# gplepage/lsqfit

Hardware: AMD Instinct MI355X
Metric: fp64 LM steps/sec at (N_data,N_param)=(65536,4096); chi2 match vs GSL (higher is better)
Workload: dtype f64

## Files before the change

lsqfit_amd/csrc/chol.hip:

```cpp
#include <cstdlib>

#include "common.h"

namespace lsqamd {

constexpr int NB = CHOL_NB;
constexpr int PLD = NB + 2;
constexpr int SB = 32;

typedef double v4d __attribute__((ext_vector_type(4)));
typedef double v2d __attribute__((ext_vector_type(2)));

size_t potrf_work_bytes(int64_t n) {
  const int64_t nblk = (n + NB - 1) / NB;
  return (size_t)nblk * NB * NB * sizeof(double);
}

__device__ __forceinline__ double readlane_d(double v, int lane) {
  union { double d; int i[2]; } u;
  u.d = v;
  u.i[0] = __builtin_amdgcn_readlane(u.i[0], lane);
  u.i[1] = __builtin_amdgcn_readlane(u.i[1], lane);
  return u.d;
}


constexpr int WLD = SB + 2;

__device__ __forceinline__ double rsqrt_refined(double d) {
  double y = __builtin_amdgcn_rsq(d);
  const double h = -0.5 * d;
  double e = __builtin_fma(h * y, y, 0.5);
  y = __builtin_fma(y, e, y);
  e = __builtin_fma(h * y, y, 0.5);
  return __builtin_fma(y, e, y);
}

__device__ __noinline__ void chol32_wave(double *s, int j0, double *dinv, double *wbuf,
                                         int32_t *info, int k0, int lane) {
  const int c = lane & 31;
  const bool isW = lane >= SB;
  double col[SB];
#pragma unroll
  for (int i = 0; i < SB; ++i) col[i] = s[(j0 + i) * PLD + j0 + c];
#pragma unroll
  for (int i = 0; i < SB; ++i) col[i] = isW ? ((i == c) ? 1.0 : 0.0) : col[i];
  int first_bad = -1;
  double d = readlane_d(col[0], 0);
  bool ok = (d > 0.0) && (d < 1.0e300);
  first_bad = ok ? first_bad : 0;
  double y = rsqrt_refined(ok ? d : 1.0);
  double ykeep = 0.0;
#pragma unroll
  for (int j = 0; j < SB; ++j) {
    double u = col[j] * y;
    u = (!isW && c < j) ? 0.0 : u;
    col[j] = u;
    ykeep = (c == j) ? y : ykeep;
    double ynext = 0.0;
    if (j + 1 < SB) {
      const double dn = readlane_d(col[j + 1] - u * u, j + 1);
      ok = (dn > 0.0) && (dn < 1.0e300);
      first_bad = (!ok && first_bad < 0) ? j + 1 : first_bad;
      ynext = rsqrt_refined(ok ? dn : 1.0);
    }
#pragma unroll
    for (int i0 = j + 1; i0 < SB; i0 += 8) {
      double ub[8];
// ... 200 lines not shown
    }
  }
  STAMP(17);
  {
    const int c2 = (tid & 63) * 2, rg = tid >> 6;
    for (int it = 0; it < 32; ++it) {
      const int r = it * 4 + rg;
      if (r >= nb) continue;
      v2d v = *reinterpret_cast<const v2d *>(s + r * PLD + c2);
      v.x = (c2 >= r && c2 < nb) ? v.x : 0.0;
      v.y = (c2 + 1 >= r && c2 + 1 < nb) ? v.y : 0.0;
      *reinterpret_cast<v2d *>(uinv + r * NB + c2) = v;
    }
  }
  STAMP(18);
}

static PerDeviceOnce g_potf2_attr;
long long *g_potf2_dbg = nullptr;
static constexpr size_t POTF2_LDS = (size_t)(NB * PLD + NB + SB * WLD) * sizeof(double);

static hipError_t launch_potf2(hipStream_t st, double *A, int64_t lda, int nb, double *uinv,
                               int32_t *info, int32_t k0, int32_t batch = 1, int64_t strideA = 0,
                               int64_t strideW = 0, const int32_t *active = nullptr) {
  {
    const hipError_t ea = g_potf2_attr.run([] {
      hipError_t e = hipFuncSetAttribute(reinterpret_cast<const void *>(potf2_inv_kernel<true>),
                                         hipFuncAttributeMaxDynamicSharedMemorySize, (int)POTF2_LDS);
      if (e != hipSuccess) return e;
      return hipFuncSetAttribute(reinterpret_cast<const void *>(potf2_inv_kernel<false>),
                                 hipFuncAttributeMaxDynamicSharedMemorySize, (int)POTF2_LDS);
    });
    if (ea != hipSuccess) return ea;
  }
  static const bool use_mfma = [] {
    const char *e = getenv("LSQAMD_POTF2");
    return !(e && e[0] == 'l');
  }();
  if (use_mfma) {
    return launch_potf2_mfma(st, A, lda, nb, uinv, info, k0, batch, strideA, strideW, active);
  }
  const bool vec = !(lda & 1) && !(reinterpret_cast<uintptr_t>(A) & 15) && !(strideA & 1);
  if (vec)
    hipLaunchKernelGGL(potf2_inv_kernel<true>, dim3((unsigned)batch), dim3(256), POTF2_LDS, st, A, lda, nb,
                       uinv, info, k0, g_potf2_dbg, strideA, strideW, active);
  else
    hipLaunchKernelGGL(potf2_inv_kernel<false>, dim3((unsigned)batch), dim3(256), POTF2_LDS, st, A, lda, nb,
                       uinv, info, k0, g_potf2_dbg, strideA, strideW, active);
  return hipGetLastError();
}

hipError_t potrf_upper_batched(hipStream_t st, double *A, int64_t n, int64_t lda, int64_t n_cols,
                               double *work, int32_t *dev_info, int32_t batch, int64_t strideA,
                               int64_t strideW, const int32_t *active, bool info_zeroed) {
  hipError_t e = info_zeroed ? hipSuccess : hipMemsetAsync(dev_info, 0, sizeof(int32_t) * (size_t)batch, st);
  if (e != hipSuccess) return e;
  static const int64_t fuse_min_tiles = [] { const char *v = getenv("LSQAMD_FUSE_MIN_TILES"); return v ? atoll(v) : (int64_t)10; }();
  const bool can_fuse = batch == 1 && !active && fuse_min_tiles >= 0 && trail_potf2_available() && (n % NB) == 0 &&
                        (n_cols % NB) == 0 &&
                        !(lda & 1) && !(reinterpret_cast<uintptr_t>(A) & 15);
  bool diag_done = false;
  for (int64_t k0 = 0; k0 < n; k0 += NB) {
    const int nb = (int)((n - k0) < NB ? (n - k0) : NB);
    double *uinv = work + (k0 / NB) * NB * NB;
    if (!diag_done) {
      e = launch_potf2(st, A + k0 * lda + k0, lda, nb, uinv, dev_info, (int32_t)k0, batch, strideA, strideW,
                       active);
      if (e != hipSuccess) return e;
    }
    diag_done = false;
    const int64_t rest = n_cols - (k0 + nb);
    if (rest <= 0) continue;
    GemmTN p;
    p.X = uinv; p.ldx = NB; p.sx = strideW;
    p.Y = A + k0 * lda + k0 + nb; p.ldy = lda; p.sy = strideA;
    p.C = A + k0 * lda + k0 + nb; p.ldc = lda; p.sc = strideA;
    p.M = nb; p.N = rest; p.K = nb;
    p.x_upper_tri = 1;
    p.batch = batch; p.batch_active = active;
    e = launch_gemm_tn(st, p);
    if (e != hipSuccess) return e;
    const int64_t mrest = n - (k0 + nb);
    if (mrest <= 0) continue;
    const int64_t tiles = (mrest / NB) * (mrest / NB + 1) / 2;
    if (can_fuse && tiles >= fuse_min_tiles) {
      e = launch_trail_potf2(st, p.C, A + (k0 + nb) * lda + (k0 + nb), lda, mrest, rest, NB,
                             work + ((k0 + nb) / NB) * NB * NB, dev_info, (int32_t)(k0 + nb));
      if (e != hipSuccess) return e;
      diag_done = true;
      continue;
    }
    GemmTN t;
    t.X = p.C; t.ldx = lda; t.sx = strideA;
    t.Y = p.C; t.ldy = lda; t.sy = strideA;
    t.C = A + (k0 + nb) * lda + (k0 + nb); t.ldc = lda; t.sc = strideA;
    t.M = mrest; t.N = rest; t.K = nb;
    t.alpha = -1.0; t.beta = 1.0;
    t.upper_only = 1;
    t.batch = batch; t.batch_active = active;
    e = launch_gemm_tn(st, t);
    if (e != hipSuccess) return e;
  }
  return hipSuccess;
}

hipError_t potrf_upper(hipStream_t st, double *A, int64_t n, int64_t lda, int64_t n_cols,
                       double *work, int32_t *dev_info, bool info_zeroed) {
  return potrf_upper_batched(st, A, n, lda, n_cols, work, dev_info, 1, 0, 0, nullptr, info_zeroed);
}

constexpr int BS_ROWS = 16;

__device__ __forceinline__ double wave_sum(double v) {
#pragma unroll
  for (int o = 32; o > 0; o >>= 1) v += __shfl_down(v, o, 64);
  return v;
}

__global__ __launch_bounds__(256) void backsolve_step_kernel(const double *A, int64_t lda, int64_t k0,
                                                             int nb, const double *uinv, double *y,
                                                             double *v, int64_t strideA, int64_t strideW,
                                                             int64_t strideY, const int32_t *active) {
  if (active && !active[blockIdx.y]) return;
  A += (int64_t)blockIdx.y * strideA;
  uinv += (int64_t)blockIdx.y * strideW;
  y += (int64_t)blockIdx.y * strideY;
  v += (int64_t)blockIdx.y * strideY;
  __shared__ double vk[NB];
  __shared__ double yk[NB];
  const int tid = threadIdx.x, lane = tid & 63, wave = tid >> 6;
  if (tid < NB) yk[tid] = tid < nb ? y[k0 + tid] : 0.0;
  double a0[32], a1[32];
#pragma unroll
  for (int i = 0; i < 32; ++i) {
    const int r = wave * 32 + i;
    const bool ok = r < nb;
    a0[i] = (ok && lane < nb) ? uinv[r * NB + lane] : 0.0;
    a1[i] = (ok && lane + 64 < nb) ? uinv[r * NB + lane + 64] : 0.0;
  }
  __syncthreads();
  const double y0 = yk[lane], y1 = yk[lane + 64];
#pragma unroll
  for (int i = 0; i < 32; ++i) {
    const double acc = wave_sum(a0[i] * y0 + a1[i] * y1);
    if (lane == 0) vk[wave * 32 + i] = acc;
  }
  __syncthreads();
  if (blockIdx.x == 0) {
    if (tid < nb) v[k0 + tid] = vk[tid];
    return;
  }
  const int64_t r0 = (int64_t)(blockIdx.x - 1) * BS_ROWS + wave * (BS_ROWS / 4);
  double u0[BS_ROWS / 4], u1[BS_ROWS / 4];
#pragma unroll
  for (int i = 0; i < BS_ROWS / 4; ++i) {
    const int64_t r = r0 + i;
    const bool ok = r < k0;
    const double *row = A + (ok ? r : 0) * lda + k0;
    u0[i] = (ok && lane < nb) ? row[lane] : 0.0;
    u1[i] = (ok && lane + 64 < nb) ? row[lane + 64] : 0.0;
  }
// ... 396 lines not shown
```

lsqfit_amd/csrc/common.h:

```cpp
#pragma once
#include <hip/hip_runtime.h>
#include <stddef.h>
#include <stdint.h>

#include <atomic>
#include <cstdio>
#include <exception>
#include <mutex>
#include <new>

#include "../../include/lsqfit_amd.h"

namespace lsqamd {

struct lsqamd_abi_no_handle { const char *err; };

template <class H> int abi_exception(H *h) noexcept {
  int code = LSQAMD_EINTERNAL;
  char buf[320];
  std::snprintf(buf, sizeof buf, "internal error: unknown C++ exception caught at the C ABI");
  try {
    throw;
  } catch (const std::bad_alloc &) {
    code = LSQAMD_ENOMEM;
// ... 69 lines not shown
  }
};

struct GemmTN {
  const double *X = nullptr, *Y = nullptr;
  double *C = nullptr;
  int64_t M = 0, N = 0, K = 0;
  int64_t ldx = 0, ldy = 0, ldc = 0;
  double alpha = 1.0, beta = 0.0;
  int32_t batch = 1;
  int64_t sx = 0, sy = 0, sc = 0;
  int32_t upper_only = 0;
  int32_t x_upper_tri = 0;
  int32_t xy_lower_tri = 0;
  int32_t splits = 1;
  int64_t split_stride = 0;
  const int32_t *work_map = nullptr;
  int32_t n_work = 0;
  int32_t force_generic = 0;
  const int32_t *batch_active = nullptr;
  int32_t tri_halves = 0;
  double *colsum_out = nullptr;
  int64_t colsum_ld = 0, colsum_rcol = 0;
  int32_t *done_ctr = nullptr;
};
bool gemm_tn_fuses_colsum(const GemmTN &g);
bool gemm_tn_wants_tri_halves(const GemmTN &g);
hipError_t launch_gemm_tn(hipStream_t st, const GemmTN &g);
struct WhitenSynth {
  int32_t model = 0;
  const double *Wt = nullptr;
  const double *x = nullptr;
  const double *p = nullptr;
  double *J = nullptr;
  int64_t ld = 0, B = 0, K = 0;
  int32_t nb = 0;
  double *colsum_out = nullptr;
  const int32_t *trig_far = nullptr;
};
bool whiten_synth_eligible(int32_t model, int64_t B, int64_t P);
hipError_t launch_whiten_synth(hipStream_t st, const WhitenSynth &a);
int64_t syrk_work_count(int64_t P, int32_t splits);
void syrk_work_fill(int64_t P, int32_t splits, int32_t *out);
int64_t syrk_work_fill_rows(int64_t P, int32_t splits, int row0, int row1, int32_t *out);
void syrk_work_fill_grouped(int64_t P, int32_t splits, int G, const int32_t *rows, int32_t *out, int32_t *count);
hipError_t launch_wait_counter(hipStream_t st, const int32_t *ctr, int32_t expect, int32_t *timed_out);

constexpr int CHOL_NB = 128;
size_t potrf_work_bytes(int64_t n);
hipError_t potrf_upper(hipStream_t st, double *A, int64_t n, int64_t lda, int64_t n_cols,
                       double *work, int32_t *dev_info, bool info_zeroed = false);
bool trail_potf2_available();
hipError_t launch_trail_potf2(hipStream_t st, const double *P, double *C, int64_t lda, int64_t mrest,
                              int64_t rest, int nb_next, double *uinv_next, int32_t *info, int32_t k0_next);
hipError_t launch_potf2_mfma(hipStream_t st, double *A, int64_t lda, int nb, double *uinv, int32_t *info,
                             int32_t k0, int32_t batch, int64_t strideA, int64_t strideW,
                             const int32_t *active);

hipError_t potrf_upper_batched(hipStream_t st, double *A, int64_t n, int64_t lda, int64_t n_cols,
                               double *work, int32_t *dev_info, int32_t batch, int64_t strideA,
                               int64_t strideW, const int32_t *active, bool info_zeroed = false);
hipError_t backsolve_upper_batched(hipStream_t st, const double *A, int64_t n, int64_t lda,
                                   const double *work, double *y_inout, int32_t batch, int64_t strideA,
                                   int64_t strideW, int64_t strideY, const int32_t *active,
                                   void *scratch = nullptr, int32_t *info_dev = nullptr, bool scratch_zeroed = false);
hipError_t trtri_upper_to_lower_T_batched(hipStream_t st, const double *A, int64_t n, int64_t lda,
                                          const double *work, double *Wl, int64_t ldw, int32_t batch,
                                          int64_t strideA, int64_t strideW, int64_t strideWl);
size_t backsolve_scratch_bytes(int64_t n);
hipError_t backsolve_upper(hipStream_t st, const double *A, int64_t n, int64_t lda,
                           const double *work, double *y_inout, void *scratch = nullptr, int32_t *info_dev = nullptr,
                           bool scratch_zeroed = false);
hipError_t trtri_upper_to_lower_T(hipStream_t st, const double *A, int64_t n, int64_t lda,
                                  const double *work, double *Wl, int64_t ldw);
hipError_t logdiag_sum(hipStream_t st, const double *A, int64_t n, int64_t lda, double *dev_out);
extern long long *g_potf2_dbg;

struct TapeProgram {
  int64_t row0 = 0, n_rows = 0;
  int32_t tape_off = 0, n_tape = 0;
  const void *jit = nullptr;
};
struct ModelArgs {
  int32_t model = 0;
  int64_t n_data = 0, n_param = 0;
  int32_t n_x = 0;
  const double *x = nullptr;
  const double *ymean = nullptr;
  const double *wdiag = nullptr;
  const uint8_t *in_block = nullptr;
  const double *p = nullptr;
  const int32_t *tape = nullptr;
  int32_t n_tape = 0;
  const double *consts = nullptr;
  int32_t n_batch = 1;
  int64_t p_stride = 0, out_stride = 0;
  int64_t ymean_stride = 0;
  int64_t wdiag_stride = 0;
  const int32_t *batch_active = nullptr;
  const int32_t *trig_far = nullptr;
  const int32_t *tape_poff = nullptr;
  double *tape_part = nullptr;
  double *tape_jt = nullptr;
  int64_t tape_ldn = 0, tape_wgs = 0;
  int32_t tape_slots = 0;
  const int32_t *tape_seg = nullptr;
  int32_t tape_n_seg = 0, tape_seg_depth = 0, tape_seg_slots = 0, tape_slot_cap = 0, tape_single = 0;
  const void *jit = nullptr;
  const TapeProgram *progs = nullptr;
  int32_t n_prog = 0;
};
int tape_slots_of_op(int op);
hipError_t launch_trig_range(hipStream_t st, const double *q, int64_t n, double xmax, int32_t *flag);
hipError_t launch_residual_ex(hipStream_t st, const ModelArgs &m, double *r_w, double *r_raw);
// ... 125 lines not shown
```

lsqfit_amd/csrc/gemm_tn_f64.hip:

```cpp
#include <cstdlib>

#include "common.h"
#include <type_traits>
#include <vector>
#include "devmath.h"

namespace lsqamd {

#ifdef LSQAMD_SYRK_STAMPS
__device__ unsigned long long *g_syrk_stamps = nullptr;
#endif

typedef double v4d __attribute__((ext_vector_type(4)));
typedef double v2d __attribute__((ext_vector_type(2)));

constexpr int BM = 128, BN = 128, BK = 16;
constexpr int LDT = BM + 16;
constexpr int STAGE = 2 * BK * LDT;
constexpr size_t GEMM_LDS_BYTES = 2 * STAGE * sizeof(double);

struct GemmDev {
  const double *X, *Y;
  double *C;
  int64_t M, N, K, ldx, ldy, ldc;
// ... 574 lines not shown
      for (int j = 0; j < 2; ++j) bb[j] = Ys[kr * LDS_S + wn * 32 + j * 16 + fr];
#pragma unroll
      for (int i = 0; i < 2; ++i)
#pragma unroll
        for (int j = 0; j < 2; ++j)
          acc[i][j] = __builtin_amdgcn_mfma_f64_16x16x4f64(a[i], bb[j], acc[i][j], 0, 0, 0);
    }
    if (more) sstore(cur ^ 1, k0 + BK);
    __syncthreads();
    cur ^= 1;
  }
  const double alpha = g.alpha;
  const double beta = g.splits > 1 ? 0.0 : g.beta;
  double cv[2][2][4];
  if (beta != 0.0) {
#pragma unroll
    for (int i = 0; i < 2; ++i)
#pragma unroll
      for (int j = 0; j < 2; ++j)
#pragma unroll
        for (int r = 0; r < 4; ++r) {
          const int64_t col = n0 + wn * 32 + j * 16 + fr;
          const int64_t row = m0 + wm * 32 + i * 16 + fq + 4 * r;
          const bool ok = col < g.N && row < g.M;
          cv[i][j][r] = C[(ok ? row : 0) * g.ldc + (ok ? col : 0)];
        }
  }
#pragma unroll
  for (int i = 0; i < 2; ++i)
#pragma unroll
    for (int j = 0; j < 2; ++j) {
      const int64_t col = n0 + wn * 32 + j * 16 + fr;
      if (col >= g.N) continue;
#pragma unroll
      for (int r = 0; r < 4; ++r) {
        const int64_t row = m0 + wm * 32 + i * 16 + fq + 4 * r;
        if (row >= g.M) continue;
        double v = alpha * acc[i][j][r];
        if (beta != 0.0) v += beta * cv[i][j][r];
        C[row * g.ldc + col] = v;
      }
    }
}

constexpr int PN = 64;
constexpr int LDS_PX = BM + 16;
constexpr int LDS_PY = PN + 16;
constexpr int STAGE_P = BK * (LDS_PX + LDS_PY);
constexpr size_t GEMM_LDS_BYTES_P = 2 * STAGE_P * sizeof(double);

constexpr int OS_LDX = 136, OS_PN = 16;
constexpr size_t GEMM_LDS_BYTES_OS = (size_t)(128 * OS_LDX + 128 * OS_PN) * sizeof(double);

__global__ __launch_bounds__(256) void gemm_tn_f64_panel_oneshot_kernel(GemmDev g) {
  extern __shared__ __attribute__((aligned(16))) double smem[];
  typedef __attribute__((address_space(3))) void lds_void;
  typedef const __attribute__((address_space(1))) void glb_void;
  const int tid = threadIdx.x, lane = tid & 63, wave = tid >> 6;
  const int64_t b = blockIdx.z;
  if (g.batch_active && !g.batch_active[b]) return;
  const double *X = g.X + b * g.sx;
  const int64_t n0 = (int64_t)blockIdx.x * OS_PN;
  double *Yg = g.C + b * g.sc + n0;
  double *Xs = smem, *Ys = smem + 128 * OS_LDX;
#pragma unroll 8
  for (int i = 0; i < 32; ++i) {
    const int k = wave * 32 + i;
    __builtin_amdgcn_global_load_lds((glb_void *)(X + (int64_t)k * g.ldx + 2 * lane), (lds_void *)(Xs + k * OS_LDX), 16, 0, 0);
  }
#pragma unroll
  for (int i = 0; i < 4; ++i) {
    const int k8 = (wave * 4 + i) * 8;
    __builtin_amdgcn_global_load_lds((glb_void *)(Yg + (int64_t)(k8 + (lane >> 3)) * g.ldc + 2 * (lane & 7)),
                                     (lds_void *)(Ys + k8 * OS_PN), 16, 0, 0);
  }
  __syncthreads();
  const int col = lane & 15, q = lane >> 4;
  const int i0 = wave, i1 = 7 - wave;
  v4d acc0 = {0.0, 0.0, 0.0, 0.0}, acc1 = {0.0, 0.0, 0.0, 0.0};
  const int n0c = 4 * (i0 + 1), n1c = 4 * (i1 + 1);
#pragma unroll 4
  for (int kc = 0; kc < n1c; ++kc) {
    const double bb = Ys[(4 * kc + q) * OS_PN + col];
    const double a1 = Xs[(4 * kc + q) * OS_LDX + 16 * i1 + col];
    acc1 = __builtin_amdgcn_mfma_f64_16x16x4f64(a1, bb, acc1, 0, 0, 0);
    if (kc < n0c) {
      const double a0 = Xs[(4 * kc + q) * OS_LDX + 16 * i0 + col];
      acc0 = __builtin_amdgcn_mfma_f64_16x16x4f64(a0, bb, acc0, 0, 0, 0);
    }
  }
#pragma unroll
  for (int r = 0; r < 4; ++r) {
    Yg[(int64_t)(16 * i0 + 4 * r + q) * g.ldc + col] = acc0[r];
    Yg[(int64_t)(16 * i1 + 4 * r + q) * g.ldc + col] = acc1[r];
  }
}

template <bool VEC, int PNW>
__global__ __launch_bounds__(256, 2) void gemm_tn_f64_panel_kernel(GemmDev g) {
  constexpr int WN = PNW >= 32 ? 2 : 1, WM = 4 / WN;
  constexpr int RW = BM / WM, NI = RW / 16;
  constexpr int CW = PNW / WN, NJ = CW / 16;
  constexpr int YT = PNW / 2, YROWS = 256 / YT;
  constexpr int YP = (BK + YROWS - 1) / YROWS;
  constexpr int LDY = PNW + 16;
  extern __shared__ __attribute__((aligned(16))) double smem[];
  const int tid = threadIdx.x;
  const int lane = tid & 63, wave = tid >> 6;
  const int wm = WN == 2 ? wave >> 1 : wave, wn = WN == 2 ? wave & 1 : 0;
  const int64_t m0 = 0, n0 = (int64_t)blockIdx.x * PNW;
  const int64_t b = blockIdx.z;
  if (g.batch_active && !g.batch_active[b]) return;
  const double *X = g.X + b * g.sx;
  const double *Y = g.Y + b * g.sy;
  double *C = g.C + b * g.sc;
  int64_t kb = 0, ke = g.K;
  if (g.x_upper_tri && ke > BM) ke = BM;
  v4d acc[NI][NJ];
#pragma unroll
  for (int i = 0; i < NI; ++i)
#pragma unroll
    for (int j = 0; j < NJ; ++j) acc[i][j] = (v4d){0.0, 0.0, 0.0, 0.0};
  const int xc2 = (tid & 63) * 2, xrg = tid >> 6;
  const int yc2 = (tid % YT) * 2, yrg = tid / YT;
  const int64_t xc = m0 + xc2, yc = n0 + yc2;
  const bool x0ok = xc < g.M, x1ok = xc + 1 < g.M;
  const bool y0ok = yc < g.N, y1ok = yc + 1 < g.N;
  const int64_t xi0 = VEC ? (xc < g.ldx - 2 ? xc : g.ldx - 2) : (xc < g.M ? xc : g.M - 1);
  const int64_t xi1 = xc + 1 < g.M ? xc + 1 : g.M - 1;
  const int64_t yi0 = VEC ? (yc < g.ldy - 2 ? yc : g.ldy - 2) : (yc < g.N ? yc : g.N - 1);
  const int64_t yi1 = yc + 1 < g.N ? yc + 1 : g.N - 1;
  v2d xr[4], yr[YP];
  auto gload = [&](int64_t k0) {
#pragma unroll
    for (int i = 0; i < 4; ++i) {
      int64_t row = k0 + xrg + 4 * i;
      row = row < ke ? row : ke - 1;
      xr[i] = load2<VEC>(X + row * g.ldx, xi0, xi1);
    }
#pragma unroll
    for (int i = 0; i < YP; ++i) {
      int64_t row = k0 + yrg + YROWS * i;
      row = row < ke ? row : ke - 1;
      yr[i] = load2<VEC>(Y + row * g.ldy, yi0, yi1);
    }
  };
  auto sstore = [&](int buf, int64_t k0) {
    double *Xs = smem + buf * STAGE_P;
// ... 622 lines not shown
```

lsqfit_amd/csrc/potf2_mfma.hip:

```cpp
#include <cstdlib>

#include "common.h"

#ifndef LSQAMD_LEAF_FMA_LAYOUT
#define LSQAMD_LEAF_FMA_LAYOUT 1
#endif

namespace lsqamd {

constexpr int NB = CHOL_NB;
typedef double v4d __attribute__((ext_vector_type(4)));

__device__ __forceinline__ double readlane_d(double v, int lane) {
  union { double d; int i[2]; } u;
  u.d = v;
  u.i[0] = __builtin_amdgcn_readlane(u.i[0], lane);
  u.i[1] = __builtin_amdgcn_readlane(u.i[1], lane);
  return u.d;
}

__device__ __forceinline__ double rsqrt_refined(double d) {
  double y = __builtin_amdgcn_rsq(d);
  const double h = -0.5 * d;
  double e = __builtin_fma(h * y, y, 0.5);
// ... 756 lines not shown
  }
}

template <int U>
__device__ __forceinline__ void tile_wave4(double *A, int64_t lda, int nb, double *uinv, Leaf4Shared &sh, int lane) {
  TileRegs4 T;
  load_tiles4<U>(T, A, lda, nb, lane);
  zero_upper_inv<U>(uinv, lane);
  Slab4Loop<0, U>::run(T, sh, A, lda, nb, uinv, lane);
}

__device__ __forceinline__ void potf2v4_run(double *A, int64_t lda, int nb, double *uinv, int32_t *info, int32_t k0,
                                            Leaf4Shared &sh, int tid) {
  const int lane = tid & 63;
  const int wave = __builtin_amdgcn_readfirstlane(tid >> 6);
  if (tid < 8) {
    sh.flagD[tid] = 0;
    sh.flagW[tid] = 0;
    sh.cnt[tid] = 0;
  }
  __syncthreads();
  if (wave == 0) pivot_wave4<true>(sh, A, lda, uinv, info, k0, nb, lane);
  else if (wave == 1) tile_wave4<0>(A, lda, nb, uinv, sh, lane);
  else if (wave == 2) tile_wave4<1>(A, lda, nb, uinv, sh, lane);
  else tile_wave4<2>(A, lda, nb, uinv, sh, lane);
}

__global__ __launch_bounds__(256) void potf2_v4_kernel(double *A, int64_t lda, int nb, double *uinv, int32_t *info,
                                                       int32_t k0, int64_t strideA, int64_t strideW,
                                                       const int32_t *active, long long *dbg) {
  __shared__ Leaf4Shared sh;
  if (active && !active[blockIdx.x]) return;
  A += (int64_t)blockIdx.x * strideA;
  uinv += (int64_t)blockIdx.x * strideW;
  info += blockIdx.x;
#ifdef LSQAMD_POTF2_TIMING
  if (threadIdx.x == 0) sh.stamps[60] = (long long)__builtin_readcyclecounter();
#endif
  potf2v4_run(A, lda, nb, uinv, info, k0, sh, threadIdx.x);
#ifdef LSQAMD_POTF2_TIMING
  __syncthreads();
  if (threadIdx.x == 0) sh.stamps[63] = (long long)__builtin_readcyclecounter();
  __syncthreads();
  if (dbg && threadIdx.x < 64) dbg[threadIdx.x] = sh.stamps[threadIdx.x];
#endif
}

struct TrailArgs {
  const double *P;
  double *C;
  int64_t lda;
  int32_t tiles_m, tiles_n;
  int32_t halves;
};

constexpr int TBK = 16, TLD = 128 + 16, TSTAGE = 2 * TBK * TLD;
constexpr size_t TRAIL_LDS_BYTES = 2 * TSTAGE * sizeof(double);

template <int NJ>
__device__ __forceinline__ void trail_tile(const TrailArgs &t, int tm, int tn, int half, double *smem, int tid) {
  const int lane = tid & 63, wave = tid >> 6;
  const int wm = wave >> 1, wn = wave & 1;
  const int64_t m0 = (int64_t)tm * 128, n0 = (int64_t)tn * 128;
  const int cw = (NJ == 4 ? 0 : 64 * half) + wn * 16 * NJ;
  v4d acc[4][NJ];
#pragma unroll
  for (int i = 0; i < 4; ++i)
#pragma unroll
    for (int j = 0; j < NJ; ++j) acc[i][j] = (v4d){0.0, 0.0, 0.0, 0.0};
  typedef __attribute__((address_space(3))) void lds_void;
  typedef const __attribute__((address_space(1))) void glb_void;
  const double *xp = t.P + (int64_t)wave * t.lda + m0 + 2 * lane;
  const double *yp = t.P + (int64_t)wave * t.lda + n0 + 2 * lane;
  const int64_t step4 = 4 * t.lda;
  auto stage = [&](int buf) {
    double *Xs = smem + buf * TSTAGE + wave * TLD;
    double *Ys = Xs + TBK * TLD;
#pragma unroll
    for (int i = 0; i < 4; ++i) {
      __builtin_amdgcn_global_load_lds((glb_void *)(xp + i * step4), (lds_void *)(Xs + 4 * i * TLD), 16, 0, 0);
      __builtin_amdgcn_global_load_lds((glb_void *)(yp + i * step4), (lds_void *)(Ys + 4 * i * TLD), 16, 0, 0);
    }
    xp += 4 * step4;
    yp += 4 * step4;
  };
  const int fr = lane & 15, fq = lane >> 4;
  stage(0);
  __syncthreads();
  int cur = 0;
  for (int k0 = 0; k0 < 128; k0 += TBK) {
    if (k0 + TBK < 128) stage(cur ^ 1);
    const double *Xs = smem + cur * TSTAGE;
    const double *Ys = Xs + TBK * TLD;
#pragma unroll
    for (int kk = 0; kk < TBK / 4; ++kk) {
      const int kr = kk * 4 + fq;
      double a[4], bb[NJ];
#pragma unroll
      for (int i = 0; i < 4; ++i) a[i] = Xs[kr * TLD + wm * 64 + i * 16 + fr];
#pragma unroll
      for (int j = 0; j < NJ; ++j) bb[j] = Ys[kr * TLD + cw + j * 16 + fr];
#pragma unroll
      for (int i = 0; i < 4; ++i)
#pragma unroll
        for (int j = 0; j < NJ; ++j) acc[i][j] = mfma4(a[i], bb[j], acc[i][j]);
    }
    __syncthreads();
    cur ^= 1;
  }
#pragma unroll
  for (int i = 0; i < 4; ++i) {
    double cv[NJ][4];
#pragma unroll
    for (int j = 0; j < NJ; ++j)
#pragma unroll
      for (int r = 0; r < 4; ++r)
        cv[j][r] = t.C[(m0 + wm * 64 + i * 16 + fq + 4 * r) * t.lda + n0 + cw + j * 16 + fr];
#pragma unroll
    for (int j = 0; j < NJ; ++j)
#pragma unroll
      for (int r = 0; r < 4; ++r)
        t.C[(m0 + wm * 64 + i * 16 + fq + 4 * r) * t.lda + n0 + cw + j * 16 + fr] = cv[j][r] - acc[i][j][r];
  }
}

constexpr int DLD4 = 128 + 8;
constexpr int DIAG4_HELP_OFF = 128 * DLD4;
constexpr size_t DIAG4_LDS_BYTES = (size_t)(128 * DLD4 + 9 * 4 * 64) * sizeof(double);
constexpr int v4_help_skip(int U) { return U == 1 ? 4 : (U == 2 ? 5 : 0); }

template <int U>
__device__ __forceinline__ void diag_update_from_panel4(TileRegs4 &T, const double *Ps, int lane) {
  const int col = lane & 15, q = lane >> 4;
#pragma unroll 4
  for (int kc = 0; kc < 32; ++kc) {
    const double *row = Ps + (4 * kc + q) * DLD4 + col;
    double a[8];
#pragma unroll
    for (int ti = 0; ti < 8; ++ti) a[ti] = -row[16 * ti];
#pragma unroll
    for (int c = 0; c < 3; ++c) {
      if (v4_has(U, c)) {
        const int tj = v4_col(U, c);
        const double b = row[16 * tj];
#pragma unroll
        for (int ti = 0; ti < 8; ++ti) {
          if (ti < tj && !(c == 2 && ti < v4_help_skip(U))) T.X[c][ti] = mfma4(a[ti], b, T.X[c][ti]);
          if (ti == tj) T.DA[c] = mfma4(a[ti], b, T.DA[c]);
        }
      }
    }
  }
}

__device__ __forceinline__ void diag_update_help4(double *Ps, int lane) {
  const int col = lane & 15, q = lane >> 4;
  const v4d zero = {0.0, 0.0, 0.0, 0.0};
  v4d h[9];
#pragma unroll
  for (int i = 0; i < 9; ++i) h[i] = zero;
#pragma unroll 4
  for (int kc = 0; kc < 32; ++kc) {
    const double *row = Ps + (4 * kc + q) * DLD4 + col;
    double a[5];
#pragma unroll
    for (int ti = 0; ti < 5; ++ti) a[ti] = -row[16 * ti];
    const double b6 = row[16 * 6], b5 = row[16 * 5];
#pragma unroll
    for (int ti = 0; ti < 4; ++ti) h[ti] = mfma4(a[ti], b6, h[ti]);
#pragma unroll
    for (int ti = 0; ti < 5; ++ti) h[4 + ti] = mfma4(a[ti], b5, h[4 + ti]);
  }
  double *help = Ps + DIAG4_HELP_OFF;
#pragma unroll
  for (int i = 0; i < 9; ++i)
#pragma unroll
    for (int r = 0; r < 4; ++r) help[(i * 4 + r) * 64 + lane] = h[i][r];
}

template <int U>
__device__ __forceinline__ void diag_update_collect4(TileRegs4 &T, const double *Ps, int lane) {
  const double *help = Ps + DIAG4_HELP_OFF;
// ... 16 lines not shown
__device__ __forceinline__ void fused_diag_wave4(const TrailArgs &t, double *Adiag, int nb, double *uinv, int32_t *info,
                                                 int32_t k0n, double *smem, int tid) {
  typedef __attribute__((address_space(3))) void lds_void;
  typedef const __attribute__((address_space(1))) void glb_void;
  const int lane = tid & 63;
#pragma unroll 8
  for (int i = 0; i < 32; ++i) {
    const int k = WV * 32 + i;
    __builtin_amdgcn_global_load_lds((glb_void *)(t.P + (int64_t)k * t.lda + 2 * lane), (lds_void *)(smem + k * DLD4), 16, 0, 0);
  }
  TileRegs4 T;
  if constexpr (WV > 0) load_tiles4<WV - 1>(T, Adiag, t.lda, nb, lane);
  __syncthreads();
  if constexpr (WV > 0) diag_update_from_panel4<WV - 1>(T, smem, lane);
  else diag_update_help4(smem, lane);
  __syncthreads();
  Leaf4Shared &sh = *reinterpret_cast<Leaf4Shared *>(smem);
  if (tid < 8) {
    sh.flagD[tid] = 0;
    sh.flagW[tid] = 0;
    sh.cnt[tid] = 0;
  }
  if constexpr (WV > 0) diag_update_collect4<WV - 1>(T, smem, lane);
  __syncthreads();
  if constexpr (WV == 0) {
    pivot_wave4<false>(sh, Adiag, t.lda, uinv, info, k0n, nb, lane);
  } else {
    if constexpr (WV == 1) publish_diag(T.DA[0], sh, 0, lane);
    zero_upper_inv<WV - 1>(uinv, lane);
    Slab4Loop<0, WV - 1>::run(T, sh, Adiag, t.lda, nb, uinv, lane);
  }
}

__global__ __launch_bounds__(256) void trail_potf2_kernel(TrailArgs t, double *Adiag, int nb, double *uinv,
                                                          int32_t *info, int32_t k0n, int pivot_wave) {
  extern __shared__ __attribute__((aligned(16))) double smem[];
  const int tid = threadIdx.x;
  [[maybe_unused]] const int lane = tid & 63;
  if (blockIdx.x > 0) {
    int rem = (int)blockIdx.x, half = 0, tm = 0;
    if (t.halves) {
      half = (rem + 1) & 1;
      rem = (rem + 1) >> 1;
    }
    while (rem >= t.tiles_n - tm) {
      rem -= t.tiles_n - tm;
      ++tm;
    }
    if (t.halves) trail_tile<2>(t, tm, tm + rem, half, smem, tid);
    else trail_tile<4>(t, tm, tm + rem, 0, smem, tid);
    return;
  }
  const int wave = __builtin_amdgcn_readfirstlane(tid >> 6);
  if (pivot_wave) {
    if (wave == 0) fused_diag_wave4<0>(t, Adiag, nb, uinv, info, k0n, smem, tid);
    else if (wave == 1) fused_diag_wave4<1>(t, Adiag, nb, uinv, info, k0n, smem, tid);
    else if (wave == 2) fused_diag_wave4<2>(t, Adiag, nb, uinv, info, k0n, smem, tid);
    else fused_diag_wave4<3>(t, Adiag, nb, uinv, info, k0n, smem, tid);
    return;
  }
}

static_assert(sizeof(Leaf4Shared) <= (size_t)128 * DLD4 * sizeof(double), "the sweep's scratch lives in the dead panel tile");
constexpr size_t TRAIL_KERNEL_LDS = TRAIL_LDS_BYTES > DIAG4_LDS_BYTES ? TRAIL_LDS_BYTES : DIAG4_LDS_BYTES;
static PerDeviceOnce g_trail_attr;

bool trail_potf2_available() {
  static const bool v4 = [] { const char *e = getenv("LSQAMD_POTF2"); return !e || (e[0] == 'v' && e[1] == '4'); }();
  return v4;
}

hipError_t launch_trail_potf2(hipStream_t st, const double *P, double *C, int64_t lda, int64_t mrest,
                              int64_t rest, int nb_next, double *uinv_next, int32_t *info, int32_t k0_next) {
  {
    const hipError_t ea = g_trail_attr.run([] {
      return hipFuncSetAttribute(reinterpret_cast<const void *>(trail_potf2_kernel),
                                 hipFuncAttributeMaxDynamicSharedMemorySize, (int)TRAIL_KERNEL_LDS);
    });
    if (ea != hipSuccess) return ea;
  }
  TrailArgs t;
  t.P = P; t.C = C; t.lda = lda;
  t.tiles_m = (int32_t)(mrest / 128);
  t.tiles_n = (int32_t)(rest / 128);
  static const int v4 = [] { const char *e = getenv("LSQAMD_POTF2"); return (!e || (e[0] == 'v' && e[1] == '4')) ? 1 : 0; }();
  const int64_t n_upper = (int64_t)t.tiles_m * t.tiles_n - (int64_t)t.tiles_m * (t.tiles_m - 1) / 2;
  static const int64_t half_from = [] { const char *e = getenv("LSQAMD_TRAIL_HALVES"); return e ? atoll(e) : (int64_t)256; }();
  t.halves = (n_upper > half_from) ? 1 : 0;
  const int64_t n_wg = t.halves ? 2 * (n_upper - 1) + 1 : n_upper;
  hipLaunchKernelGGL(trail_potf2_kernel, dim3((unsigned)n_wg), dim3(256), TRAIL_KERNEL_LDS,
                     st, t, C, nb_next, uinv_next, info, k0_next, v4);
  return hipGetLastError();
}

hipError_t launch_potf2_mfma(hipStream_t st, double *A, int64_t lda, int nb, double *uinv, int32_t *info,
                             int32_t k0, int32_t batch, int64_t strideA, int64_t strideW,
                             const int32_t *active) {
  static const bool v2 = [] { const char *e = getenv("LSQAMD_POTF2"); return e && e[0] == 'v' && e[1] == '2'; }();
  static const bool v4 = [] { const char *e = getenv("LSQAMD_POTF2"); return !e || (e[0] == 'v' && e[1] == '4'); }();
  if (v4)
    hipLaunchKernelGGL(potf2_v4_kernel, dim3((unsigned)batch), dim3(256), 0, st, A, lda, nb, uinv, info, k0, strideA,
                       strideW, active, g_potf2_dbg);
  else if (v2)
    hipLaunchKernelGGL(potf2_mfma_kernel, dim3((unsigned)batch), dim3(256), 0, st, A, lda, nb, uinv, info,
                       k0, strideA, strideW, active);
  else
    hipLaunchKernelGGL(potf2_v3_kernel, dim3((unsigned)batch), dim3(256), 0, st, A, lda, nb, uinv, info,
                       k0, strideA, strideW, active, g_potf2_dbg);
  return hipGetLastError();
}

}
```

Baseline: 53.87.

## Fold next diagonal block update into panel solve kernel for small trailing matrices

For late Cholesky steps with small trailing matrices, the trailing-update kernel now saves a pristine copy of the next panel's first off-diagonal tile into extra workspace. The panel triangular-solve kernel then also updates the next diagonal block from it, using extra workgroups that run MFMA products on 16x16 sub-tiles. The following trail kernel can then skip its in-kernel diagonal update and just factor the block. The goal is to take the diagonal update off the critical path of the fused trail+potf2 kernel. In exchange the panel solve is recomputed per sub-tile pair, one more workspace block is allocated, and correctness now relies on the helper-tile conventions of the pivot wave.

```diff
diff --git a/lsqfit_amd/csrc/chol.hip b/lsqfit_amd/csrc/chol.hip
--- a/lsqfit_amd/csrc/chol.hip
+++ b/lsqfit_amd/csrc/chol.hip
@@ -13,7 +13,7 @@
 
 size_t potrf_work_bytes(int64_t n) {
   const int64_t nblk = (n + NB - 1) / NB;
-  return (size_t)nblk * NB * NB * sizeof(double);
+  return (size_t)(nblk + 1) * NB * NB * sizeof(double);
 }
 
 __device__ __forceinline__ double readlane_d(double v, int lane) {
@@ -320,13 +320,23 @@
 
 hipError_t potrf_upper_batched(hipStream_t st, double *A, int64_t n, int64_t lda, int64_t n_cols,
                                double *work, int32_t *dev_info, int32_t batch, int64_t strideA,
-                               int64_t strideW, const int32_t *active, bool info_zeroed) {
+                               int64_t strideW, const int32_t *active, bool info_zeroed, bool work_has_scratch) {
   hipError_t e = info_zeroed ? hipSuccess : hipMemsetAsync(dev_info, 0, sizeof(int32_t) * (size_t)batch, st);
   if (e != hipSuccess) return e;
   static const int64_t fuse_min_tiles = [] { const char *v = getenv("LSQAMD_FUSE_MIN_TILES"); return v ? atoll(v) : (int64_t)10; }();
   const bool can_fuse = batch == 1 && !active && fuse_min_tiles >= 0 && trail_potf2_available() && (n % NB) == 0 &&
                         (n_cols % NB) == 0 &&
                         !(lda & 1) && !(reinterpret_cast<uintptr_t>(A) & 15);
+  const char *dip_env = getenv("LSQAMD_DIAG_IN_PANEL");
+  const char *dip_max_env = getenv("LSQAMD_DIAG_IN_PANEL_MAX_TILES");
+  const int64_t dip_max_tiles = dip_max_env ? atoll(dip_max_env) : (int64_t)240;
+  const bool diag_in_panel = can_fuse && work_has_scratch && !(dip_env && dip_env[0] == '0') &&
+                             panel_oneshot_diag_available() && !(reinterpret_cast<uintptr_t>(work) & 15);
+  double *pristine = work + ((n + NB - 1) / NB) * NB * NB;
+  auto fused_at = [&](int64_t k) {
+    const int64_t mb = (n - (k + NB)) / NB;
+    return can_fuse && mb > 0 && mb * (mb + 1) / 2 >= fuse_min_tiles && mb * (mb + 1) / 2 <= dip_max_tiles;
+  };
   bool diag_done = false;
   for (int64_t k0 = 0; k0 < n; k0 += NB) {
     const int nb = (int)((n - k0) < NB ? (n - k0) : NB);
@@ -336,6 +346,7 @@
                        active);
       if (e != hipSuccess) return e;
     }
+    const bool next_in_panel = diag_in_panel && diag_done && fused_at(k0);
     diag_done = false;
     const int64_t rest = n_cols - (k0 + nb);
     if (rest <= 0) continue;
@@ -346,14 +357,16 @@
     p.M = nb; p.N = rest; p.K = nb;
     p.x_upper_tri = 1;
     p.batch = batch; p.batch_active = active;
-    e = launch_gemm_tn(st, p);
+    if (next_in_panel) e = launch_panel_oneshot_diag(st, uinv, p.C, lda, rest, pristine, A + (k0 + nb) * lda + (k0 + nb));
+    else e = launch_gemm_tn(st, p);
     if (e != hipSuccess) return e;
     const int64_t mrest = n - (k0 + nb);
     if (mrest <= 0) continue;
     const int64_t tiles = (mrest / NB) * (mrest / NB + 1) / 2;
     if (can_fuse && tiles >= fuse_min_tiles) {
       e = launch_trail_potf2(st, p.C, A + (k0 + nb) * lda + (k0 + nb), lda, mrest, rest, NB,
-                             work + ((k0 + nb) / NB) * NB * NB, dev_info, (int32_t)(k0 + nb));
+                             work + ((k0 + nb) / NB) * NB * NB, dev_info, (int32_t)(k0 + nb),
+                             (diag_in_panel && fused_at(k0 + nb)) ? pristine : nullptr, next_in_panel);
       if (e != hipSuccess) return e;
       diag_done = true;
       continue;
@@ -374,7 +387,7 @@
 
 hipError_t potrf_upper(hipStream_t st, double *A, int64_t n, int64_t lda, int64_t n_cols,
                        double *work, int32_t *dev_info, bool info_zeroed) {
-  return potrf_upper_batched(st, A, n, lda, n_cols, work, dev_info, 1, 0, 0, nullptr, info_zeroed);
+  return potrf_upper_batched(st, A, n, lda, n_cols, work, dev_info, 1, 0, 0, nullptr, info_zeroed, true);
 }
 
 constexpr int BS_ROWS = 16;
diff --git a/lsqfit_amd/csrc/common.h b/lsqfit_amd/csrc/common.h
--- a/lsqfit_amd/csrc/common.h
+++ b/lsqfit_amd/csrc/common.h
@@ -145,14 +145,20 @@
                        double *work, int32_t *dev_info, bool info_zeroed = false);
 bool trail_potf2_available();
 hipError_t launch_trail_potf2(hipStream_t st, const double *P, double *C, int64_t lda, int64_t mrest,
-                              int64_t rest, int nb_next, double *uinv_next, int32_t *info, int32_t k0_next);
+                              int64_t rest, int nb_next, double *uinv_next, int32_t *info, int32_t k0_next,
+                              double *pristine_out = nullptr, bool diag_updated = false);
+constexpr bool potf2_diag_helper_block(int ti, int tj) { return (tj == 6 && ti < 4) || (tj == 5 && ti < 5); }
+bool panel_oneshot_diag_available();
+hipError_t launch_panel_oneshot_diag(hipStream_t st, const double *uinv, double *panel, int64_t lda, int64_t rest,
+                                     const double *pristine, double *Dnext);
 hipError_t launch_potf2_mfma(hipStream_t st, double *A, int64_t lda, int nb, double *uinv, int32_t *info,
                              int32_t k0, int32_t batch, int64_t strideA, int64_t strideW,
                              const int32_t *active);
 
 hipError_t potrf_upper_batched(hipStream_t st, double *A, int64_t n, int64_t lda, int64_t n_cols,
                                double *work, int32_t *dev_info, int32_t batch, int64_t strideA,
-                               int64_t strideW, const int32_t *active, bool info_zeroed = false);
+                               int64_t strideW, const int32_t *active, bool info_zeroed = false,
+                               bool work_has_scratch = false);
 hipError_t backsolve_upper_batched(hipStream_t st, const double *A, int64_t n, int64_t lda,
                                    const double *work, double *y_inout, int32_t batch, int64_t strideA,
                                    int64_t strideW, int64_t strideY, const int32_t *active,
diff --git a/lsqfit_amd/csrc/gemm_tn_f64.hip b/lsqfit_amd/csrc/gemm_tn_f64.hip
--- a/lsqfit_amd/csrc/gemm_tn_f64.hip
+++ b/lsqfit_amd/csrc/gemm_tn_f64.hip
@@ -650,32 +650,33 @@
 constexpr int OS_LDX = 136, OS_PN = 16;
 constexpr size_t GEMM_LDS_BYTES_OS = (size_t)(128 * OS_LDX + 128 * OS_PN) * sizeof(double);
 
-__global__ __launch_bounds__(256) void gemm_tn_f64_panel_oneshot_kernel(GemmDev g) {
-  extern __shared__ __attribute__((aligned(16))) double smem[];
+__device__ __forceinline__ void oneshot_stage_x(const double *X, int64_t ldx, double *Xs, int wave, int lane) {
   typedef __attribute__((address_space(3))) void lds_void;
   typedef const __attribute__((address_space(1))) void glb_void;
-  const int tid = threadIdx.x, lane = tid & 63, wave = tid >> 6;
-  const int64_t b = blockIdx.z;
-  if (g.batch_active && !g.batch_active[b]) return;
-  const double *X = g.X + b * g.sx;
-  const int64_t n0 = (int64_t)blockIdx.x * OS_PN;
-  double *Yg = g.C + b * g.sc + n0;
-  double *Xs = smem, *Ys = smem + 128 * OS_LDX;
 #pragma unroll 8
   for (int i = 0; i < 32; ++i) {
     const int k = wave * 32 + i;
-    __builtin_amdgcn_global_load_lds((glb_void *)(X + (int64_t)k * g.ldx + 2 * lane), (lds_void *)(Xs + k * OS_LDX), 16, 0, 0);
-  }
+    __builtin_amdgcn_global_load_lds((glb_void *)(X + (int64_t)k * ldx + 2 * lane), (lds_void *)(Xs + k * OS_LDX), 16, 0, 0);
+  }
+}
+
+__device__ __forceinline__ void oneshot_stage_y(const double *Yg, int64_t ldy, double *Ys, int wave, int lane) {
+  typedef __attribute__((address_space(3))) void lds_void;
+  typedef const __attribute__((address_space(1))) void glb_void;
 #pragma unroll
   for (int i = 0; i < 4; ++i) {
     const int k8 = (wave * 4 + i) * 8;
-    __builtin_amdgcn_global_load_lds((glb_void *)(Yg + (int64_t)(k8 + (lane >> 3)) * g.ldc + 2 * (lane & 7)),
+    __builtin_amdgcn_global_load_lds((glb_void *)(Yg + (int64_t)(k8 + (lane >> 3)) * ldy + 2 * (lane & 7)),
                                      (lds_void *)(Ys + k8 * OS_PN), 16, 0, 0);
   }
-  __syncthreads();
+}
+
+__device__ __forceinline__ void oneshot_product(const double *Xs, const double *Ys, int wave, int lane, v4d &acc0,
+                                                v4d &acc1) {
   const int col = lane & 15, q = lane >> 4;
   const int i0 = wave, i1 = 7 - wave;
-  v4d acc0 = {0.0, 0.0, 0.0, 0.0}, acc1 = {0.0, 0.0, 0.0, 0.0};
+  acc0 = (v4d){0.0, 0.0, 0.0, 0.0};
+  acc1 = (v4d){0.0, 0.0, 0.0, 0.0};
   const int n0c = 4 * (i0 + 1), n1c = 4 * (i1 + 1);
 #pragma unroll 4
   for (int kc = 0; kc < n1c; ++kc) {
@@ -687,11 +688,141 @@
       acc0 = __builtin_amdgcn_mfma_f64_16x16x4f64(a0, bb, acc0, 0, 0, 0);
     }
   }
+}
+
+__device__ __forceinline__ void oneshot_slice(const double *X, int64_t ldx, double *Yg, int64_t ldc, double *smem,
+                                              int tid) {
+  const int lane = tid & 63, wave = tid >> 6;
+  double *Xs = smem, *Ys = smem + 128 * OS_LDX;
+  oneshot_stage_x(X, ldx, Xs, wave, lane);
+  oneshot_stage_y(Yg, ldc, Ys, wave, lane);
+  __syncthreads();
+  const int col = lane & 15, q = lane >> 4;
+  const int i0 = wave, i1 = 7 - wave;
+  v4d acc0, acc1;
+  oneshot_product(Xs, Ys, wave, lane, acc0, acc1);
 #pragma unroll
   for (int r = 0; r < 4; ++r) {
-    Yg[(int64_t)(16 * i0 + 4 * r + q) * g.ldc + col] = acc0[r];
-    Yg[(int64_t)(16 * i1 + 4 * r + q) * g.ldc + col] = acc1[r];
-  }
+    Yg[(int64_t)(16 * i0 + 4 * r + q) * ldc + col] = acc0[r];
+    Yg[(int64_t)(16 * i1 + 4 * r + q) * ldc + col] = acc1[r];
+  }
+}
+
+__global__ __launch_bounds__(256) void gemm_tn_f64_panel_oneshot_kernel(GemmDev g) {
+  extern __shared__ __attribute__((aligned(16))) double smem[];
+  const int64_t b = blockIdx.z;
+  if (g.batch_active && !g.batch_active[b]) return;
+  oneshot_slice(g.X + b * g.sx, g.ldx, g.C + b * g.sc + (int64_t)blockIdx.x * OS_PN, g.ldc, smem, threadIdx.x);
+}
+
+constexpr int PD_PAIRS = 36;
+
+struct PanelDiagArgs {
+  const double *X;
+  double *Y;
+  int64_t ldc;
+  const double *pristine;
+  double *D;
+};
+
+__global__ __launch_bounds__(256) void gemm_tn_f64_panel_oneshot_diag_kernel(PanelDiagArgs g) {
+  extern __shared__ __attribute__((aligned(16))) double smem[];
+  const int tid = threadIdx.x, lane = tid & 63;
+  const int wave = __builtin_amdgcn_readfirstlane(tid >> 6);
+  if (blockIdx.x >= PD_PAIRS) {
+    oneshot_slice(g.X, CHOL_NB, g.Y + (int64_t)(blockIdx.x - PD_PAIRS) * OS_PN, g.ldc, smem, tid);
+    return;
+  }
+  int ti = (int)blockIdx.x, tj = 0;
+  while (ti > tj) {
+    ti -= tj + 1;
+    ++tj;
+  }
+  const int col = lane & 15, q = lane >> 4;
+  double *Xs = smem, *Ys = smem + 128 * OS_LDX;
+  oneshot_stage_x(g.X, CHOL_NB, Xs, wave, lane);
+  oneshot_stage_y(g.pristine + 16 * tj, CHOL_NB, Ys, wave, lane);
+  v2d y2[4];
+  if (ti != tj) {
+#pragma unroll
+    for (int i = 0; i < 4; ++i) {
+      const int k8 = (wave * 4 + i) * 8;
+      y2[i] = *reinterpret_cast<const v2d *>(g.pristine + (int64_t)(k8 + (lane >> 3)) * CHOL_NB + 16 * ti + 2 * (lane & 7));
+    }
+  }
+  v4d c = {0.0, 0.0, 0.0, 0.0};
+  if (wave == 0) {
+#pragma unroll
+    for (int r = 0; r < 4; ++r) c[r] = g.D[(int64_t)(16 * ti + 4 * r + q) * g.ldc + 16 * tj + col];
+  }
+  __syncthreads();
+  const int i0 = wave, i1 = 7 - wave;
+  v4d acc0, acc1;
+  double a[32], b[32];
+  auto solved_to_lds = [&]() {
+    __syncthreads();
+#pragma unroll
+    for (int r = 0; r < 4; ++r) {
+      Ys[(16 * i0 + 4 * r + q) * OS_PN + col] = acc0[r];
+      Ys[(16 * i1 + 4 * r + q) * OS_PN + col] = acc1[r];
+    }
+    __syncthreads();
+  };
+  oneshot_product(Xs, Ys, wave, lane, acc0, acc1);
+  solved_to_lds();
+  if (wave == 0) {
+#pragma unroll
+    for (int kc = 0; kc < 32; ++kc) b[kc] = Ys[(4 * kc + q) * OS_PN + col];
+  }
+  if (ti != tj) {
+    __syncthreads();
+#pragma unroll
+    for (int i = 0; i < 4; ++i) {
+      const int k8 = (wave * 4 + i) * 8;
+      *reinterpret_cast<v2d *>(Ys + (k8 + (lane >> 3)) * OS_PN + 2 * (lane & 7)) = y2[i];
+    }
+    __syncthreads();
+    oneshot_product(Xs, Ys, wave, lane, acc0, acc1);
+    solved_to_lds();
+    if (wave == 0) {
+#pragma unroll
+      for (int kc = 0; kc < 32; ++kc) a[kc] = -Ys[(4 * kc + q) * OS_PN + col];
+    }
+  } else if (wave == 0) {
+#pragma unroll
+    for (int kc = 0; kc < 32; ++kc) a[kc] = -b[kc];
+  }
+  if (wave != 0) return;
+  const bool helper = potf2_diag_helper_block(ti, tj);
+  v4d acc = helper ? (v4d){0.0, 0.0, 0.0, 0.0} : c;
+#pragma unroll
+  for (int kc = 0; kc < 32; ++kc) acc = __builtin_amdgcn_mfma_f64_16x16x4f64(a[kc], b[kc], acc, 0, 0, 0);
+  if (helper) {
+#pragma unroll
+    for (int r = 0; r < 4; ++r) acc[r] = c[r] + acc[r];
+  }
+#pragma unroll
+  for (int r = 0; r < 4; ++r) g.D[(int64_t)(16 * ti + 4 * r + q) * g.ldc + 16 * tj + col] = acc[r];
+}
+
+bool panel_oneshot_diag_available() {
+  static const bool ok = [] { const char *e = getenv("LSQAMD_PANEL_PN"); return !(e && atoi(e) != 0); }();
+  return ok;
+}
+
+hipError_t launch_panel_oneshot_diag(hipStream_t st, const double *uinv, double *panel, int64_t lda, int64_t rest,
+                                     const double *pristine, double *Dnext) {
+  static PerDeviceOnce attr;
+  const hipError_t ea = attr.run([] {
+    return hipFuncSetAttribute(reinterpret_cast<const void *>(gemm_tn_f64_panel_oneshot_diag_kernel),
+                               hipFuncAttributeMaxDynamicSharedMemorySize, (int)GEMM_LDS_BYTES_OS);
+  });
+  if (ea != hipSuccess) return ea;
+  PanelDiagArgs g;
+  g.X = uinv; g.Y = panel; g.ldc = lda; g.pristine = pristine; g.D = Dnext;
+  hipLaunchKernelGGL(gemm_tn_f64_panel_oneshot_diag_kernel, dim3((unsigned)(PD_PAIRS + rest / OS_PN)), dim3(256),
+                     GEMM_LDS_BYTES_OS, st, g);
+  return hipGetLastError();
 }
 
 template <bool VEC, int PNW>
diff --git a/lsqfit_amd/csrc/potf2_mfma.hip b/lsqfit_amd/csrc/potf2_mfma.hip
--- a/lsqfit_amd/csrc/potf2_mfma.hip
+++ b/lsqfit_amd/csrc/potf2_mfma.hip
@@ -832,6 +832,8 @@
   int64_t lda;
   int32_t tiles_m, tiles_n;
   int32_t halves;
+  int32_t diag_updated;
+  double *pristine;
 };
 
 constexpr int TBK = 16, TLD = 128 + 16, TSTAGE = 2 * TBK * TLD;
@@ -901,6 +903,13 @@
 #pragma unroll
       for (int r = 0; r < 4; ++r)
         t.C[(m0 + wm * 64 + i * 16 + fq + 4 * r) * t.lda + n0 + cw + j * 16 + fr] = cv[j][r] - acc[i][j][r];
+    if (t.pristine && tm == 0 && tn == 1) {
+#pragma unroll
+      for (int j = 0; j < NJ; ++j)
+#pragma unroll
+        for (int r = 0; r < 4; ++r)
+          t.pristine[(wm * 64 + i * 16 + fq + 4 * r) * NB + cw + j * 16 + fr] = cv[j][r] - acc[i][j][r];
+    }
   }
 }
 
@@ -908,6 +917,9 @@
 constexpr int DIAG4_HELP_OFF = 128 * DLD4;
 constexpr size_t DIAG4_LDS_BYTES = (size_t)(128 * DLD4 + 9 * 4 * 64) * sizeof(double);
 constexpr int v4_help_skip(int U) { return U == 1 ? 4 : (U == 2 ? 5 : 0); }
+static_assert(potf2_diag_helper_block(3, 6) && !potf2_diag_helper_block(4, 6) && potf2_diag_helper_block(4, 5) &&
+              !potf2_diag_helper_block(5, 5) && !potf2_diag_helper_block(0, 7) && v4_help_skip(1) == 4 && v4_help_skip(2) == 5,
+              "potf2_diag_helper_block (common.h) names the pivot wave's helper tiles");
 
 template <int U>
 __device__ __forceinline__ void diag_update_from_panel4(TileRegs4 &T, const double *Ps, int lane) {
@@ -1030,6 +1042,10 @@
     return;
   }
   const int wave = __builtin_amdgcn_readfirstlane(tid >> 6);
+  if (t.diag_updated) {
+    potf2v4_run(Adiag, t.lda, nb, uinv, info, k0n, *reinterpret_cast<Leaf4Shared *>(smem), tid);
+    return;
+  }
   if (pivot_wave) {
     if (wave == 0) fused_diag_wave4<0>(t, Adiag, nb, uinv, info, k0n, smem, tid);
     else if (wave == 1) fused_diag_wave4<1>(t, Adiag, nb, uinv, info, k0n, smem, tid);
@@ -1049,7 +1065,8 @@
 }
 
 hipError_t launch_trail_potf2(hipStream_t st, const double *P, double *C, int64_t lda, int64_t mrest,
-                              int64_t rest, int nb_next, double *uinv_next, int32_t *info, int32_t k0_next) {
+                              int64_t rest, int nb_next, double *uinv_next, int32_t *info, int32_t k0_next,
+                              double *pristine_out, bool diag_updated) {
   {
     const hipError_t ea = g_trail_attr.run([] {
       return hipFuncSetAttribute(reinterpret_cast<const void *>(trail_potf2_kernel),
@@ -1061,10 +1078,12 @@
   t.P = P; t.C = C; t.lda = lda;
   t.tiles_m = (int32_t)(mrest / 128);
   t.tiles_n = (int32_t)(rest / 128);
+  t.pristine = t.tiles_n >= 2 ? pristine_out : nullptr;
   static const int v4 = [] { const char *e = getenv("LSQAMD_POTF2"); return (!e || (e[0] == 'v' && e[1] == '4')) ? 1 : 0; }();
   const int64_t n_upper = (int64_t)t.tiles_m * t.tiles_n - (int64_t)t.tiles_m * (t.tiles_m - 1) / 2;
   static const int64_t half_from = [] { const char *e = getenv("LSQAMD_TRAIL_HALVES"); return e ? atoll(e) : (int64_t)256; }();
   t.halves = (n_upper > half_from) ? 1 : 0;
+  t.diag_updated = (diag_updated && v4) ? 1 : 0;
   const int64_t n_wg = t.halves ? 2 * (n_upper - 1) + 1 : n_upper;
   hipLaunchKernelGGL(trail_potf2_kernel, dim3((unsigned)n_wg), dim3(256), TRAIL_KERNEL_LDS,
                      st, t, C, nb_next, uinv_next, info, k0_next, v4);
```

Result: faster. 54.43, median of 6 (+1.0%).
